# alibaba/graph-learn

Hardware: AMD Instinct MI355X
Metric: sampled-edges/sec + aggregated-vertices/sec (2-hop sample + aggregate per step) (higher is better)
Workload: dtype f32

## Files before the change

### graph-learn_amd/csrc/glx_aggregate.hip

```cpp
#include <float.h>
#include <stdlib.h>
#include <string.h>

#include <atomic>
#include <mutex>
#include <new>
#include <type_traits>

#include "glx_common.h"

namespace {

constexpr int32_t kSegRunMax = 64;


__global__ void glx_seg_reset_kernel(unsigned long long* words) {
  words[0] = 0;
  words[1] = 0;
}

__global__ __launch_bounds__(256) void glx_seg_scan_kernel(const int32_t* __restrict__ seg, int32_t n, int32_t num_segments,
                                                           int32_t f, unsigned long long* __restrict__ words, uint32_t epoch,
                                                           int32_t* __restrict__ seg_start) {
  const int64_t i0 = ((int64_t)blockIdx.x * blockDim.x + threadIdx.x) * 4;
  if (i0 >= n) return;
  int32_t v[4];
  const int32_t m = (n - i0) < 4 ? (int32_t)(n - i0) : 4;
  if (m == 4 && (reinterpret_cast<uintptr_t>(seg) & 15) == 0) {
    const int4 q = *reinterpret_cast<const int4*>(seg + i0);
    v[0] = q.x; v[1] = q.y; v[2] = q.z; v[3] = q.w;
  } else {
    for (int j = 0; j < 4; ++j) v[j] = j < m ? seg[i0 + j] : 0;
  }
  int32_t prev = i0 > 0 ? seg[i0 - 1] : -1;
  if (i0 > 0 && (prev < 0 || prev >= num_segments)) return;
  int32_t quo = f > 0 ? (int32_t)(i0 / f) : 0, rem = f > 0 ? (int32_t)(i0 % f) : 0;
  bool nonuniform = false, incomplete = false;
  int32_t bad_at = n;
  for (int j = 0; j < m; ++j) {
    const int32_t i = (int32_t)i0 + j, cur = v[j];
    if (cur < 0 || cur >= num_segments || cur < prev) {
      bad_at = i;
      break;
    }
    if (cur != prev) {
      if (cur - prev > kSegRunMax) incomplete = true;
      else for (int32_t s = prev + 1; s <= cur; ++s) seg_start[s] = i;
    }
    if (f > 0) {
      nonuniform |= cur != quo;
      if (++rem == f) { rem = 0; ++quo; }
    }
    prev = cur;
  }
  if (bad_at == n && i0 + m == n) {
    if (num_segments - prev > kSegRunMax) incomplete = true;
    else for (int32_t s = prev + 1; s <= num_segments; ++s) seg_start[s] = n;
  }
  const unsigned long long tag = (unsigned long long)epoch << 32;
  if (bad_at < n) atomicMax(&words[0], tag | (uint32_t)(n - bad_at));
  const int32_t level = (incomplete || bad_at < n) ? 2 : (nonuniform ? 1 : 0);
  const uint64_t here = __ballot(true), at2 = __ballot(level == 2), at1 = __ballot(level >= 1);
  const int32_t wave_level = at2 ? 2 : (at1 ? 1 : 0);
  if (wave_level && (threadIdx.x & 63) == (unsigned)(__ffsll((long long)here) - 1)) {
    const unsigned long long mine = tag | (uint32_t)wave_level;
    if (__hip_atomic_load(&words[1], __ATOMIC_RELAXED, __HIP_MEMORY_SCOPE_AGENT) < mine) atomicMax(&words[1], mine);
  }
}

__global__ void glx_seg_fixup_kernel(const int32_t* __restrict__ seg, SegState st, int32_t n, int32_t num_segments,
                                     int32_t* __restrict__ seg_start) {
  if (seg_level(st) != 2) return;
  int32_t s = blockIdx.x * blockDim.x + threadIdx.x;
  if (s > num_segments) return;
  int32_t lo = 0, hi = seg_valid_len(st, n);
  while (lo < hi) {
    int32_t mid = lo + ((hi - lo) >> 1);
    if (seg[mid] < s) lo = mid + 1; else hi = mid;
  }
  seg_start[s] = lo;
}

__global__ void glx_rows_kernel(GlxIdMap map, const int64_t* __restrict__ ids, int64_t n,
                                int32_t* __restrict__ rows) {
  int64_t i = blockIdx.x * (int64_t)blockDim.x + threadIdx.x;
  if (i >= n) return;
  rows[i] = (int32_t)glx_row_of(map, ids[i]);
}


__host__ __device__ __forceinline__ uint16_t glx_f32_to_bf16_bits(uint32_t u) {
  if ((u & 0x7fffffffu) > 0x7f800000u) return 0xFFFF;
  return (uint16_t)((u + 0x7FFFu + ((u >> 16) & 1u)) >> 16);
}
__host__ __device__ __forceinline__ uint16_t glx_f32_to_f16_bits(uint32_t u) {
  const uint32_t sign = (u >> 16) & 0x8000u;
  const uint32_t a = u & 0x7fffffffu;
  if (a > 0x7f800000u) return (uint16_t)(sign | 0x7E00u | ((a >> 13) & 0x3FFu));
  if (a >= 0x477FF000u) return (uint16_t)(sign | 0x7C00u);
  if (a >= 0x38800000u) {
    const uint32_t m = a - 0x38000000u;
    return (uint16_t)(sign | ((m + 0xFFFu + ((m >> 13) & 1u)) >> 13));
  }
  const uint32_t e = a >> 23;
  const uint32_t sh = 126u - e;
  if (sh >= 25u) return (uint16_t)sign;
  const uint32_t mant = (a & 0x7fffffu) | 0x800000u;
  const uint32_t q = mant >> sh, rem = mant & ((1u << sh) - 1u), half = 1u << (sh - 1u);
  return (uint16_t)(sign | (q + ((rem > half || (rem == half && (q & 1u))) ? 1u : 0u)));
}

struct AggArgs {
  const void* X;
  const int64_t* node_ids;
  const int32_t* rows;
  const int32_t* seg_start;
  SegState seg_state;
  float* emb_out;
  int32_t* cnt_out;
  int64_t num_rows;
  int64_t stride;
  int64_t swizzle_rows;
  int32_t dim;
  int32_t num_segments;
  int32_t fanout;
  float default_attr;
  int32_t col0, ncols;
  int32_t store_mode;
  int32_t load_repeats;
  int32_t segs_per_group;
  int32_t xcd_slices;
  int32_t stripe_chunk;
  uint32_t stripe_full;
  const float* X1;
  const float* X2;
  int64_t stride1, swizzle1, stride2;
  int32_t base1, base2;
  int32_t dtype;
};

__device__ __forceinline__ int32_t agg_row_at(const AggArgs& a, int32_t pos) {
  if (a.rows) return a.rows[pos];
  const int64_t id = a.node_ids[pos];
  return (id >= 0 && id < a.num_rows) ? (int32_t)id : -1;
}

template <int NSRC, int DT = GLX_DTYPE_F32>
__device__ __forceinline__ const typename AggElem<DT>::raw* agg_row_ptr(const AggArgs& a, int32_t row) {
  const typename AggElem<DT>::raw* X = static_cast<const typename AggElem<DT>::raw*>(a.X);
  if constexpr (NSRC == 1) {
    return X + glx_swizzle_row(row, a.swizzle_rows) * a.stride;
  } else {
    static_assert(DT == GLX_DTYPE_F32, "the distributed store's row sources are float32");
    if (row < a.base1) return X + glx_swizzle_row(row, a.swizzle_rows) * a.stride;
    if (row < a.base2) return a.X1 + glx_swizzle_row(row - a.base1, a.swizzle1) * a.stride1;
    return a.X2 + (int64_t)(row - a.base2) * a.stride2;
  }
}

template <int OP, int G, int VEC, int U, int NSRC, int DT>
__global__ __launch_bounds__(256) void glx_aggregate_kernel(AggArgs a) {
  typedef float vec_t __attribute__((ext_vector_type(VEC)));
  const int64_t gid = (blockIdx.x * (int64_t)blockDim.x + threadIdx.x) / G;
  const int c = threadIdx.x & (G - 1);
  if (gid >= a.num_segments) return;
  int32_t s0, s1;
  if (a.seg_start && seg_level(a.seg_state) != 0) {
    s0 = a.seg_start[gid];
    s1 = a.seg_start[gid + 1];
  } else {
    s0 = (int32_t)gid * a.fanout;
    s1 = s0 + a.fanout;
  }
  const int32_t n = s1 - s0;
  if (c == 0 && a.col0 == 0) a.cnt_out[gid] = n;
  float* out = a.emb_out + gid * (int64_t)a.dim;
  const int32_t col_end = a.col0 + a.ncols;
  for (int32_t col = a.col0 + c * VEC; col < col_end; col += G * VEC) {
    vec_t acc;
#pragma unroll
    for (int v = 0; v < VEC; ++v) acc[v] = agg_init<OP>();
    for (int32_t base = s0; base < s1; base += U) {
      int32_t row[U];
#pragma unroll
      for (int u = 0; u < U; ++u) row[u] = (base + u < s1) ? agg_row_at(a, base + u) : -2;
      vec_t val[U];
#pragma unroll
      for (int u = 0; u < U; ++u) {
        if (row[u] >= 0) {
          val[u] = agg_load<DT, VEC>(agg_row_ptr<NSRC, DT>(a, row[u]) + col);
        } else {
#pragma unroll
          for (int v = 0; v < VEC; ++v) val[u][v] = a.default_attr;
        }
      }
#pragma unroll
      for (int u = 0; u < U; ++u) {
        if (row[u] != -2) {
#pragma unroll
          for (int v = 0; v < VEC; ++v) acc[v] = agg_combine<OP>(acc[v], val[u][v]);
        }
      }
    }
    if (n == 0) {
#pragma unroll
      for (int v = 0; v < VEC; ++v) acc[v] = a.default_attr;
    } else if (OP == GLX_AGG_MEAN) {
      const float fn = (float)n;
#pragma unroll
      for (int v = 0; v < VEC; ++v) acc[v] = acc[v] / fn;
    }
    *reinterpret_cast<vec_t*>(out + col) = acc;
  }
}

template <int G, int IDR>
__device__ __forceinline__ void agg_chunk_load(const AggArgs& a, int32_t chunk_base, int32_t pos_end, int c,
                                               int32_t (&myrow)[IDR]) {
#pragma unroll
  for (int k = 0; k < IDR; ++k) {
    const int32_t pos = chunk_base + k * G + c;
    myrow[k] = pos < pos_end ? agg_row_at(a, pos) : -1;
  }
}

template <int G, int IDR>
__device__ __forceinline__ int32_t agg_chunk_get(const int32_t (&myrow)[IDR], int32_t idx) {
  if (G == 64) {
    int32_t r = __builtin_amdgcn_readlane(myrow[0], idx & 63);
#pragma unroll
    for (int k = 1; k < IDR; ++k) {
      const int32_t t = __builtin_amdgcn_readlane(myrow[k], idx & 63);
      r = (idx >> 6) == k ? t : r;
// ... 187 lines not shown
          folded = true;
        }
      }
      for (int32_t base = s0; !folded && base < s1; base += U) {
        const int32_t stop = (s1 - base) < U ? s1 : base + U;
        if (stop > chunk_base + kChunk) {
          chunk_base = base;
          agg_chunk_load<G, IDR>(a, chunk_base, pos_end, c, myrow);
        }
        if (stop - base == U) agg_grp_batch<OP, G, VEC, U, NSRC, IDR, true, DT>(a, myrow, base - chunk_base, U, col_ld, acc);
        else agg_grp_batch<OP, G, VEC, U, NSRC, IDR, false, DT>(a, myrow, base - chunk_base, stop - base, col_ld, acc);
      }
      const int32_t n = s1 - s0;
      if (n == 0) {
#pragma unroll
        for (int v = 0; v < VEC; ++v) acc[v] = a.default_attr;
      } else if (OP == GLX_AGG_MEAN) {
        const float fn = (float)n;
#pragma unroll
        for (int v = 0; v < VEC; ++v) acc[v] = acc[v] / fn;
      }
      if (col_ok) {
        float* const dst = a.emb_out + sg * (int64_t)a.dim + col;
        if constexpr (VEC == 8) {
          agg_store4(a.store_mode, dst, acc.lo);
          agg_store4(a.store_mode, dst + 4, acc.hi);
        } else {
          if (a.store_mode == 1) *reinterpret_cast<vec_t*>(dst) = acc;
          else __builtin_nontemporal_store(acc, reinterpret_cast<vec_t*>(dst));
        }
      }
      if (c == 0 && col_pass == 0) a.cnt_out[sg] = n;
    }
  }
}

__device__ __forceinline__ bool agg_nonfinite4(float __attribute__((ext_vector_type(4))) v) {
  const uint32_t e = 0x7f800000u;
  return ((__float_as_uint(v[0]) & e) == e) || ((__float_as_uint(v[1]) & e) == e) || ((__float_as_uint(v[2]) & e) == e) ||
         ((__float_as_uint(v[3]) & e) == e);
}

__device__ __noinline__ float agg_mfma_serial(const float* X, const int64_t* node_ids, const int32_t* rows,
                                              int64_t num_rows, int64_t stride, int64_t swizzle_rows,
                                              float default_attr, int64_t sg, int32_t col, int32_t f) {
  float acc = 0.0f;
  for (int32_t r = 0; r < f; ++r) {
    const int64_t pos = sg * f + r;
    int64_t row;
    if (rows) {
      row = rows[pos];
    } else {
      const int64_t id = node_ids[pos];
      row = (id >= 0 && id < num_rows) ? id : -1;
    }
    const float x = row >= 0 ? X[glx_swizzle_row(row, swizzle_rows) * stride + col] : default_attr;
    acc = acc + x;
  }
  return acc;
}

template <int OP, int NB>
__global__ __launch_bounds__(256) void glx_aggregate_mfma_kernel(AggArgs a) {
  typedef float f4 __attribute__((ext_vector_type(4)));
  constexpr int KC = 32;
  extern __shared__ float tile[];
  constexpr int32_t D = 64 * NB;
  constexpr int32_t pitch = D + 16;
  const int32_t f = a.fanout;
  const int64_t seg0 = (int64_t)blockIdx.x * 16;
  const int32_t nseg = (int32_t)((a.num_segments - seg0) < 16 ? (a.num_segments - seg0) : 16);
  const int64_t id0 = seg0 * f;
  const int32_t nrows = nseg * f;
  const int lane = threadIdx.x & 63;
  const int wave = threadIdx.x >> 6;
  const int m = lane & 15;
  const int kq = lane >> 4;
  f4 acc[NB];
#pragma unroll
  for (int b = 0; b < NB; ++b) acc[b] = f4{0.f, 0.f, 0.f, 0.f};
  constexpr int32_t row_f4 = D / 4;
  constexpr int32_t PT = KC * row_f4 / 256;
  bool nonfinite = false;
  for (int32_t base = 0; base < nrows; base += KC) {
    f4 v[PT];
#pragma unroll
    for (int i = 0; i < PT; ++i) {
      const int32_t p = threadIdx.x + i * 256;
      const int32_t r = p / row_f4;
      const int32_t c4 = p - r * row_f4;
      v[i] = f4{0.f, 0.f, 0.f, 0.f};
      if (base + r < nrows) {
        const int32_t row = agg_row_at(a, (int32_t)(id0 + base + r));
        if (row >= 0) v[i] = *reinterpret_cast<const f4*>(agg_row_ptr<1>(a, row) + c4 * 4);
        else v[i] = f4{a.default_attr, a.default_attr, a.default_attr, a.default_attr};
      }
    }
#pragma unroll
    for (int i = 0; i < PT; ++i) {
      const int32_t p = threadIdx.x + i * 256;
      const int32_t r = p / row_f4;
      const int32_t c4 = p - r * row_f4;
      *reinterpret_cast<f4*>(tile + r * pitch + c4 * 4) = v[i];
      nonfinite |= agg_nonfinite4(v[i]);
    }
    __syncthreads();
#pragma unroll 2
    for (int32_t k4 = 0; k4 < KC; k4 += 4) {
      const int32_t krow = base + k4 + kq;
      const float ind = (krow < nrows && krow / f == m) ? 1.0f : 0.0f;
      const float* brow = tile + (k4 + kq) * pitch + wave * (D / 4) + m;
#pragma unroll
      for (int b = 0; b < NB; ++b) {
        acc[b] = __builtin_amdgcn_mfma_f32_16x16x4f32(ind, brow[b * 16], acc[b], 0, 0, 0);
      }
    }
    __syncthreads();
  }
  const bool refold = __syncthreads_or(nonfinite) != 0;
#pragma unroll
  for (int reg = 0; reg < 4; ++reg) {
    const int32_t srow = kq * 4 + reg;
    if (srow < nseg) {
      float* out = a.emb_out + (seg0 + srow) * (int64_t)D + wave * (D / 4) + m;
#pragma unroll
      for (int b = 0; b < NB; ++b) {
        float v = acc[b][reg];
        if (refold) {
          v = agg_mfma_serial(static_cast<const float*>(a.X), a.node_ids, a.rows, a.num_rows, a.stride, a.swizzle_rows,
                              a.default_attr, seg0 + srow, wave * (D / 4) + m + b * 16, f);
        }
        if (f == 0) v = a.default_attr;
        else if (OP == GLX_AGG_MEAN) v = v / (float)f;
        out[b * 16] = v;
      }
    }
  }
  if (threadIdx.x < nseg) a.cnt_out[seg0 + threadIdx.x] = f;
}

struct AggKnobs {
  std::atomic<int> mfma{0};
  std::atomic<int> unroll{0};
  std::atomic<int> slices{0};
  std::atomic<int> legacy{0};
  std::atomic<int> segs{0};
  std::atomic<int> xcd{0};
  std::atomic<int> occ{0};
  std::atomic<int> store{0};
  std::atomic<int> stripes{-1};
  std::atomic<int> chunk{0};
  std::atomic<int> half_ld16{0};
  std::atomic<int> repeats{0};
};

AggKnobs& agg_knobs() {
  static AggKnobs k;
  static std::once_flag once;
  std::call_once(once, [] {
    auto env = [](const char* name) {
      const char* e = getenv(name);
      return e ? atoi(e) : 0;
    };
    k.mfma = env("GLX_AGG_MFMA");
    k.unroll = env("GLX_AGG_UNROLL");
    k.slices = env("GLX_AGG_SLICES");
    k.legacy = env("GLX_AGG_LEGACY");
    k.segs = env("GLX_AGG_SEGS");
    k.xcd = env("GLX_AGG_XCD_SLICES");
    k.occ = env("GLX_AGG_OCCUPANCY");
    k.store = env("GLX_AGG_STORE");
    if (getenv("GLX_AGG_XCD_STRIPES")) k.stripes = env("GLX_AGG_XCD_STRIPES");
    k.chunk = env("GLX_AGG_XCD_CHUNK");
    k.half_ld16 = env("GLX_AGG_HALF_LD16");
    k.repeats = env("GLX_AGG_REPEATS");
  });
  return k;
}

bool agg_use_mfma(const AggArgs& a, int op) {
  if (agg_knobs().mfma.load(std::memory_order_relaxed) == 0) return false;
  return a.dtype == GLX_DTYPE_F32 && (op == GLX_AGG_SUM || op == GLX_AGG_MEAN) && a.seg_start == nullptr && a.fanout > 0 && a.X1 == nullptr &&
         a.X2 == nullptr && (a.dim == 64 || a.dim == 128 || a.dim == 256) && (a.stride % 4) == 0 &&
         (reinterpret_cast<uintptr_t>(a.X) & 15) == 0;
}

template <int OP>
void launch_agg_mfma(const AggArgs& a, hipStream_t s) {
  const unsigned grid = (unsigned)((a.num_segments + 15) / 16);
  const size_t lds = (size_t)32 * (a.dim + 16) * sizeof(float);
  if (a.dim == 64) glx_aggregate_mfma_kernel<OP, 1><<<grid, 256, lds, s>>>(a);
  else if (a.dim == 128) glx_aggregate_mfma_kernel<OP, 2><<<grid, 256, lds, s>>>(a);
  else glx_aggregate_mfma_kernel<OP, 4><<<grid, 256, lds, s>>>(a);
}

template <int OP, int G, int VEC, int NSRC, int DT>
void launch_agg_g(const AggArgs& a, hipStream_t s) {
  const int64_t threads = (int64_t)a.num_segments * G;
  const unsigned grid = (unsigned)((threads + 255) / 256);
  constexpr bool kWide = VEC == 4 && G >= 32;
  glx_aggregate_kernel<OP, G, VEC, kWide ? 6 : 8, NSRC, DT><<<grid, 256, 0, s>>>(a);
}

int agg_grp_unroll(int32_t fanout, int32_t avg_len) {
  static const int kU[] = {6, 8, 10, 12, 15};
  const int want = agg_knobs().unroll.load(std::memory_order_relaxed);
  for (int u : kU) {
    if (u == want) return u;
  }
  const int32_t f = fanout > 0 ? fanout : (avg_len > 0 ? avg_len : 10);
  int best = 10, best_batches = INT32_MAX;
  for (int u : kU) {
    const int batches = (f + u - 1) / u;
    if (batches < best_batches) {
      best = u;
      best_batches = batches;
    }
  }
  return best;
}

constexpr int32_t kAggSkipMinLen = 16;

template <int OP, int G, int VEC, int NSRC, int IDR, int DT>
void launch_agg_grp(AggArgs a, int32_t num_ids, hipStream_t s) {
  const int32_t avg = a.num_segments > 0 ? (int32_t)(num_ids / a.num_segments) : 0;
  int32_t S = 1;
  const int want = agg_knobs().segs.load(std::memory_order_relaxed);
  constexpr int64_t kElemBytes = sizeof(typename AggElem<DT>::raw);
  if (NSRC == 1 && (int64_t)a.num_rows * a.stride * kElemBytes <= ((int64_t)1 << 30) && a.num_segments >= 3 * 32768) S = 3;
  if (want > 0) S = want;
  if (S > G - 1) S = G - 1;
  if (S < 1) S = 1;
  a.segs_per_group = S;
  a.store_mode = agg_knobs().store.load(std::memory_order_relaxed);
  const int repeats = agg_knobs().repeats.load(std::memory_order_relaxed);
  a.load_repeats = repeats == 1 ? 1 : (repeats == 2 ? 0 : (avg >= kAggSkipMinLen ? 0 : 1));
  const int64_t groups = ((int64_t)a.num_segments + S - 1) / S;
  const int64_t seg_blocks = (groups + (256 / G) - 1) / (256 / G);
  const int32_t nsl = a.xcd_slices > 1 ? a.xcd_slices : 1;
  const int64_t blocks = seg_blocks * nsl;
  const unsigned grid = (unsigned)blocks;
  if (a.stripe_chunk > 0 && nsl < 8) {
    const int64_t span = (int64_t)(8 / nsl) * a.stripe_chunk;
    a.stripe_full = (uint32_t)(seg_blocks / span * span);
  } else {
    a.stripe_chunk = 0;
    a.stripe_full = 0;
  }
  const int occ = agg_knobs().occ.load(std::memory_order_relaxed);
  const size_t lds = (occ >= 3 && occ <= 7) ? (size_t)(160 * 1024 / occ) & ~(size_t)255 : 0;
  switch (agg_grp_unroll(a.seg_start ? 0 : a.fanout, avg)) {
    case 6: glx_aggregate_grp_kernel<OP, G, VEC, 6, NSRC, IDR, DT><<<grid, 256, lds, s>>>(a); break;
    case 8: glx_aggregate_grp_kernel<OP, G, VEC, 8, NSRC, IDR, DT><<<grid, 256, lds, s>>>(a); break;
    case 12: glx_aggregate_grp_kernel<OP, G, VEC, 12, NSRC, IDR, DT><<<grid, 256, lds, s>>>(a); break;
    case 15: glx_aggregate_grp_kernel<OP, G, VEC, 15, NSRC, IDR, DT><<<grid, 256, lds, s>>>(a); break;
    default: glx_aggregate_grp_kernel<OP, G, VEC, 10, NSRC, IDR, DT><<<grid, 256, lds, s>>>(a); break;
  }
}

template <int OP, int VEC, int NSRC, int DT>
void launch_agg_grp_g(const AggArgs& a, int lanes, int32_t num_ids, hipStream_t s) {
  if (lanes >= 64) launch_agg_grp<OP, 64, VEC, NSRC, 1, DT>(a, num_ids, s);
  else if (lanes >= 32) launch_agg_grp<OP, 32, VEC, NSRC, 1, DT>(a, num_ids, s);
  else if (lanes >= 16) launch_agg_grp<OP, 16, VEC, NSRC, 1, DT>(a, num_ids, s);
  else launch_agg_grp<OP, 8, VEC, NSRC, 2, DT>(a, num_ids, s);
}

template <int OP, int NSRC, int DT>
void launch_agg_cols(const AggArgs& a0, int32_t num_ids, int want_xcd, hipStream_t s) {
  AggArgs a = a0;
  bool vec4 = a.dim % 4 == 0 && a.ncols % 4 == 0 && a.col0 % 4 == 0 && (reinterpret_cast<uintptr_t>(a.emb_out) & 15) == 0 &&
              (reinterpret_cast<uintptr_t>(a.X) & 15) == 0 && (a.stride % 4) == 0;
  if (NSRC > 1) {
    vec4 = vec4 && (reinterpret_cast<uintptr_t>(a.X1) & 15) == 0 && (reinterpret_cast<uintptr_t>(a.X2) & 15) == 0 &&
           (a.stride1 % 4) == 0 && (a.stride2 % 4) == 0;
  }
  const int ev = (DT != GLX_DTYPE_F32 && agg_knobs().half_ld16.load(std::memory_order_relaxed) != 0) ? 8 : 4;
  const bool wide = vec4 && a.dim % ev == 0 && a.ncols % ev == 0 && a.col0 % ev == 0 && (a.stride % ev) == 0;
  const bool has_rows = NSRC > 1 ? (a.X2 != nullptr || a.base2 > 0) : a.num_rows > 0;
  if (wide && has_rows && a.ncols >= 8 * ev && agg_knobs().legacy.load(std::memory_order_relaxed) == 0) {
    if (want_xcd > 1 && a.col0 == 0 && a.ncols == a.dim && a.dim % (ev * want_xcd) == 0 && a.dim / want_xcd >= 8 * ev) {
      a.xcd_slices = want_xcd;
      a.ncols = a.dim / want_xcd;
    }
    if constexpr (DT != GLX_DTYPE_F32) {
      if (ev == 8) {
        launch_agg_grp_g<OP, 8, NSRC, DT>(a, a.ncols / 8, num_ids, s);
        return;
      }
    }
    launch_agg_grp_g<OP, 4, NSRC, DT>(a, a.ncols / 4, num_ids, s);
    return;
  }
  if (vec4) {
    const int lanes = a.ncols / 4;
    if (lanes >= 64) launch_agg_g<OP, 64, 4, NSRC, DT>(a, s);
    else if (lanes >= 32) launch_agg_g<OP, 32, 4, NSRC, DT>(a, s);
    else if (lanes >= 16) launch_agg_g<OP, 16, 4, NSRC, DT>(a, s);
    else if (lanes >= 8) launch_agg_g<OP, 8, 4, NSRC, DT>(a, s);
    else if (lanes >= 4) launch_agg_g<OP, 4, 4, NSRC, DT>(a, s);
    else if (lanes >= 2) launch_agg_g<OP, 2, 4, NSRC, DT>(a, s);
    else launch_agg_g<OP, 1, 4, NSRC, DT>(a, s);
  } else {
    const int lanes = a.ncols;
    if (lanes >= 64) launch_agg_g<OP, 64, 1, NSRC, DT>(a, s);
    else if (lanes >= 16) launch_agg_g<OP, 16, 1, NSRC, DT>(a, s);
    else if (lanes >= 4) launch_agg_g<OP, 4, 1, NSRC, DT>(a, s);
    else launch_agg_g<OP, 1, 1, NSRC, DT>(a, s);
  }
}

constexpr int32_t kXcdSliceMinIds = 4 << 20;
constexpr int32_t kXcdStripeChunk = 64;

template <int OP, int NSRC, int DT>
void launch_agg_n(const AggArgs& a0, int32_t num_ids, hipStream_t s) {
  AggArgs a = a0;
  a.col0 = 0;
  a.ncols = a.dim;
  a.xcd_slices = 0;
  int stripes = agg_knobs().stripes.load(std::memory_order_relaxed);
  if (stripes < 0) stripes = num_ids >= kXcdSliceMinIds ? 1 : 0;
  int xcd = agg_knobs().xcd.load(std::memory_order_relaxed);
  if (xcd == 0) {
    xcd = (num_ids >= kXcdSliceMinIds && a.dim % 8 == 0 && a.dim >= 128) ? 2 : 1;
    if (xcd == 2 && stripes > 0 && a.dim >= 256) xcd = 1;
  }
  int slices = agg_knobs().slices.load(std::memory_order_relaxed);
  if ((slices != 2 && slices != 4 && slices != 8) || a.dim % (4 * slices) != 0) slices = 1;
  if (xcd != 2 && xcd != 4 && xcd != 8) xcd = 1;
  int chunk = agg_knobs().chunk.load(std::memory_order_relaxed);
  if (chunk <= 0) chunk = kXcdStripeChunk;
  a.stripe_chunk = stripes > 0 ? chunk : 0;
  for (int c = 0; c < slices; ++c) {
    a.ncols = a.dim / slices;
    a.col0 = c * a.ncols;
    launch_agg_cols<OP, NSRC, DT>(a, num_ids, slices == 1 ? xcd : 1, s);
  }
}

template <int OP>
void launch_agg(const AggArgs& a, int32_t num_ids, hipStream_t s) {
  if (a.X1 || a.X2) launch_agg_n<OP, 3, GLX_DTYPE_F32>(a, num_ids, s);
  else if (a.dtype == GLX_DTYPE_BF16) launch_agg_n<OP, 1, GLX_DTYPE_BF16>(a, num_ids, s);
  else if (a.dtype == GLX_DTYPE_F16) launch_agg_n<OP, 1, GLX_DTYPE_F16>(a, num_ids, s);
  else launch_agg_n<OP, 1, GLX_DTYPE_F32>(a, num_ids, s);
}

template <int SRC, int DST>
__global__ void glx_place_rows_kernel(const void* __restrict__ src_v, int64_t num_rows, int32_t dim,
                                      int64_t stride, int64_t swizzle_rows, void* __restrict__ dst_v) {
  typedef typename std::conditional<SRC == GLX_DTYPE_F32, uint32_t, uint16_t>::type src_t;
  typedef typename std::conditional<DST == GLX_DTYPE_F32, uint32_t, uint16_t>::type dst_t;
  const src_t* __restrict__ src = static_cast<const src_t*>(src_v);
  dst_t* __restrict__ dst = static_cast<dst_t*>(dst_v);
  const int64_t total = num_rows * (int64_t)dim;
  const int64_t step = (int64_t)gridDim.x * blockDim.x;
  for (int64_t t = blockIdx.x * (int64_t)blockDim.x + threadIdx.x; t < total; t += step) {
    const int64_t r = t / dim;
    const int32_t c = (int32_t)(t - r * dim);
    dst_t v;
    if constexpr (SRC == DST) v = src[t];
    else if constexpr (DST == GLX_DTYPE_BF16) v = glx_f32_to_bf16_bits(src[t]);
    else v = glx_f32_to_f16_bits(src[t]);
    dst[glx_swizzle_row(r, swizzle_rows) * stride + c] = v;
  }
}

template <int DT>
__global__ __launch_bounds__(256) void glx_lookup_kernel(GlxIdMap map, const void* __restrict__ Xv,
                                                         int64_t stride, int64_t swizzle_rows, int32_t dim, const int64_t* __restrict__ ids,
                                                         int64_t n, float default_attr,
                                                         float* __restrict__ out, int G) {
  const typename AggElem<DT>::raw* __restrict__ X = static_cast<const typename AggElem<DT>::raw*>(Xv);
  const int64_t gid = (blockIdx.x * (int64_t)blockDim.x + threadIdx.x) / G;
  const int c = threadIdx.x % G;
  if (gid >= n) return;
  int64_t row = glx_row_of(map, ids[gid]);
  if (row >= 0) row = glx_swizzle_row(row, swizzle_rows);
  float* o = out + gid * (int64_t)dim;
  bool vec4 = (dim & 3) == 0;
  if constexpr (DT != GLX_DTYPE_F32) vec4 = vec4 && (stride & 3) == 0 && (reinterpret_cast<uintptr_t>(Xv) & 7) == 0;
  if (vec4) {
    for (int32_t col = c * 4; col < dim; col += G * 4) {
      float4 v = make_float4(default_attr, default_attr, default_attr, default_attr);
      if (row >= 0) {
        const float __attribute__((ext_vector_type(4))) q = agg_load<DT, 4>(X + row * stride + col);
        v = make_float4(q[0], q[1], q[2], q[3]);
      }
      *reinterpret_cast<float4*>(o + col) = v;
    }
  } else {
    for (int32_t col = c; col < dim; col += G) o[col] = row >= 0 ? AggElem<DT>::up(X[row * stride + col]) : default_attr;
  }
}

int run_aggregate(AggArgs& a, int op, const int32_t* d_seg, int32_t num_ids, hipStream_t s) {
  GlxKernelTimer timer(GLX_KERNEL_AGGREGATE, s);
  if (agg_use_mfma(a, op)) {
    if (op == GLX_AGG_SUM) launch_agg_mfma<GLX_AGG_SUM>(a, s);
    else launch_agg_mfma<GLX_AGG_MEAN>(a, s);
    timer.stop();
    return GLX_OK;
  }
  switch (op) {
    case GLX_AGG_SUM: launch_agg<GLX_AGG_SUM>(a, num_ids, s); break;
    case GLX_AGG_MEAN: launch_agg<GLX_AGG_MEAN>(a, num_ids, s); break;
    case GLX_AGG_MAX: launch_agg<GLX_AGG_MAX>(a, num_ids, s); break;
    case GLX_AGG_MIN: launch_agg<GLX_AGG_MIN>(a, num_ids, s); break;
    case GLX_AGG_PROD: launch_agg<GLX_AGG_PROD>(a, num_ids, s); break;
    default: break;
  }
  timer.stop();
  return GLX_OK;
}

namespace {
struct SegBuf {
  int dev;
  hipStream_t stream;
  unsigned long long* words;
  uint32_t epoch;
};
constexpr size_t kSegBufsMax = 64;
struct SegWords {
  std::vector<SegBuf> bufs;
  ~SegWords() {
    for (auto& e : bufs) {
      if (hipSetDevice(e.dev) == hipSuccess) (void)hipFree(e.words);
    }
    (void)hipGetLastError();
  }
};
thread_local SegWords g_seg_words;

int seg_words_for(hipStream_t s, unsigned long long** out, uint32_t* epoch) {
  int dev = 0;
  GLX_HIP(hipGetDevice(&dev));
  SegBuf* buf = nullptr;
  for (auto& e : g_seg_words.bufs) {
    if (e.dev == dev && e.stream == s) {
      buf = &e;
      break;
    }
  }
  if (buf == nullptr) {
    if (g_seg_words.bufs.size() >= kSegBufsMax) {
      const SegBuf old = g_seg_words.bufs.front();
      g_seg_words.bufs.erase(g_seg_words.bufs.begin());
      GlxDeviceGuard guard(old.dev);
      (void)hipFree(old.words);
    }
    unsigned long long* p = nullptr;
    GLX_HIP(hipMalloc(&p, 256));
    GLX_HIP(hipMemsetAsync(p, 0, 256, s));
    g_seg_words.bufs.push_back(SegBuf{dev, s, p, 0u});
    buf = &g_seg_words.bufs.back();
  }
  if (++buf->epoch == 0) {
    GLX_HIP(hipMemsetAsync(buf->words, 0, 16, s));
    buf->epoch = 1;
  }
  *out = buf->words;
  *epoch = buf->epoch;
  return GLX_OK;
}
}


int prepare_segments(AggArgs& a, const int32_t* d_seg, int32_t num_ids, int32_t num_segments, int32_t* scratch,
                     hipStream_t s) {
  a.fanout = num_segments > 0 ? num_ids / num_segments : 0;
  memset(&a.seg_state, 0, sizeof(a.seg_state));
  if (d_seg == nullptr) {
    a.seg_start = nullptr;
    return GLX_OK;
  }
  int32_t* seg_start = scratch;
  unsigned long long* words = nullptr;
  SegState st;
  hipStreamCaptureStatus capturing = hipStreamCaptureStatusNone;
  if (hipStreamIsCapturing(s, &capturing) == hipSuccess && capturing != hipStreamCaptureStatusNone) {
    const uintptr_t at = (reinterpret_cast<uintptr_t>(scratch + (size_t)num_segments + 1) + 7) & ~(uintptr_t)7;
    words = reinterpret_cast<unsigned long long*>(at);
    st.epoch = 1;
    glx_seg_reset_kernel<<<1, 1, 0, s>>>(words);
  } else {
    int rc = seg_words_for(s, &words, &st.epoch);
    if (rc != GLX_OK) return rc;
  }
  const int32_t f = (num_segments > 0 && num_ids > 0 && num_ids % num_segments == 0) ? num_ids / num_segments : 0;
  st.words = words;
  st.floor_level = num_ids == 0 ? 2 : (f > 0 ? 0 : 1);
  if (num_ids > 0) {
    glx_seg_scan_kernel<<<(unsigned)(((int64_t)num_ids + 1023) / 1024), 256, 0, s>>>(d_seg, num_ids, num_segments, f, words,
                                                                                   st.epoch, seg_start);
  }
  glx_seg_fixup_kernel<<<(unsigned)((num_segments + 1 + 255) / 256), 256, 0, s>>>(d_seg, st, num_ids, num_segments, seg_start);
  a.seg_start = seg_start;
  a.seg_state = st;
  return GLX_OK;
}

int aggregate_device(const glx_features* f, int op, const int64_t* d_ids, const int32_t* d_seg,
                     int32_t num_ids, int32_t num_segments, float default_attr, float* d_emb,
                     int32_t* d_cnt, hipStream_t s) {
  const bool hashed = f->idmap.any();
  const size_t n_i32 = (size_t)num_segments + 1 + kSegScratchExtra + (hashed ? (size_t)num_ids : 0);
  GlxScratch lease;
  int rc = lease.alloc(n_i32 * sizeof(int32_t), s, 1);
  if (rc != GLX_OK) return rc;
  int32_t* scratch = lease.as<int32_t>();
  int32_t* rows = hashed ? scratch + num_segments + 1 + kSegScratchExtra : nullptr;
  AggArgs a;
  memset(&a, 0, sizeof(a));
  rc = prepare_segments(a, d_seg, num_ids, num_segments, scratch, s);
  if (rc != GLX_OK) return rc;
  if (hashed && num_ids > 0) {
    glx_rows_kernel<<<(unsigned)((num_ids + 255) / 256), 256, 0, s>>>(f->map(), d_ids, num_ids, rows);
  }
  a.X = f->X;
  a.dtype = f->dtype;
  a.node_ids = hashed ? nullptr : d_ids;
  a.rows = rows;
  a.emb_out = d_emb;
  a.cnt_out = d_cnt;
  a.num_rows = f->num_rows;
  a.stride = f->stride;
  a.swizzle_rows = f->swizzle_rows;
  a.dim = f->dim;
  a.num_segments = num_segments;
  a.default_attr = default_attr;
  run_aggregate(a, op, d_seg, num_ids, s);
  GLX_HIP(hipGetLastError());
  return GLX_OK;
}

template <int OP, int VEC>
__global__ __launch_bounds__(256) void glx_agg_stitch_kernel(const float* __restrict__ parts,
                                                             const int32_t* __restrict__ cnts, int32_t P,
                                                             int64_t num_segments, int32_t dim,
                                                             float default_attr, float* __restrict__ out,
                                                             int32_t* __restrict__ cnt_out) {
  const int32_t cols = dim / VEC;
  const int64_t t = blockIdx.x * (int64_t)blockDim.x + threadIdx.x;
  if (t >= num_segments * cols) return;
  const int64_t sg = t / cols;
  const int32_t c0 = (int32_t)(t - sg * cols) * VEC;
  float acc[VEC];
#pragma unroll
  for (int v = 0; v < VEC; ++v) acc[v] = agg_init<OP>();
  int32_t total = 0;
  for (int32_t p = 0; p < P; ++p) {
    const int32_t c = cnts[(int64_t)p * num_segments + sg];
    if (c == 0) continue;
    const float* src = parts + ((int64_t)p * num_segments + sg) * dim + c0;
    float r[VEC];
    if (VEC == 4) {
      const float4 q = *reinterpret_cast<const float4*>(src);
      r[0] = q.x; r[1 % VEC] = q.y; r[2 % VEC] = q.z; r[3 % VEC] = q.w;
    } else {
      r[0] = src[0];
    }
#pragma unroll
    for (int v = 0; v < VEC; ++v) {
      const float x = OP == GLX_AGG_MEAN ? r[v] * (float)c : r[v];
      acc[v] = agg_combine<OP>(acc[v], x);
    }
    total += c;
  }
#pragma unroll
  for (int v = 0; v < VEC; ++v) {
    if (total == 0) acc[v] = default_attr;
    else if (OP == GLX_AGG_MEAN) acc[v] = acc[v] / (float)total;
  }
  float* dst = out + sg * dim + c0;
  if (VEC == 4) *reinterpret_cast<float4*>(dst) = make_float4(acc[0], acc[1 % VEC], acc[2 % VEC], acc[3 % VEC]);
  else dst[0] = acc[0];
  if (c0 == 0) cnt_out[sg] = total;
}

template <int OP>
void launch_agg_stitch(bool vec4, const float* parts, const int32_t* cnts, int32_t P, int64_t sg, int32_t dim,
                       float default_attr, float* out, int32_t* cnt_out, hipStream_t s) {
  const int64_t threads = sg * (vec4 ? dim / 4 : dim);
  const unsigned grid = (unsigned)((threads + 255) / 256);
  if (vec4) glx_agg_stitch_kernel<OP, 4><<<grid, 256, 0, s>>>(parts, cnts, P, sg, dim, default_attr, out, cnt_out);
  else glx_agg_stitch_kernel<OP, 1><<<grid, 256, 0, s>>>(parts, cnts, P, sg, dim, default_attr, out, cnt_out);
}

}

int glx_aggregate_vrows_device(const GlxRowSource* src, int nsrc, int32_t dim, int op, const int32_t* vrows,
                               const int32_t* d_seg, int32_t num_ids, int32_t num_segments, float default_attr,
                               float* d_emb, int32_t* d_cnt, hipStream_t s) {
  GlxScratch lease;
  int rc = lease.alloc(((size_t)num_segments + 1 + kSegScratchExtra) * sizeof(int32_t), s, 1);
  if (rc != GLX_OK) return rc;
  int32_t* scratch = lease.as<int32_t>();
  AggArgs a;
  memset(&a, 0, sizeof(a));
  rc = prepare_segments(a, d_seg, num_ids, num_segments, scratch, s);
  if (rc != GLX_OK) return rc;
  const GlxRowSource none{nullptr, dim, 0, 0};
  const GlxRowSource& s0 = nsrc > 0 ? src[0] : none;
  const GlxRowSource& s1 = nsrc > 1 ? src[1] : none;
  const GlxRowSource& s2 = nsrc > 2 ? src[2] : none;
  a.X = s0.X;
  a.stride = s0.stride;
  a.swizzle_rows = s0.swizzle_rows;
  a.num_rows = s0.rows;
  a.X1 = s1.X;
  a.stride1 = s1.stride;
  a.swizzle1 = s1.swizzle_rows;
  a.X2 = s2.X;
  a.stride2 = s2.stride;
  a.base1 = (int32_t)s0.rows;
  a.base2 = (int32_t)(s0.rows + s1.rows);
  a.node_ids = nullptr;
  a.rows = vrows;
  a.emb_out = d_emb;
  a.cnt_out = d_cnt;
  a.dim = dim;
  a.num_segments = num_segments;
  a.default_attr = default_attr;
  run_aggregate(a, op, d_seg, num_ids, s);
  GLX_HIP(hipGetLastError());
  return GLX_OK;
}

int glx_segments_prepare(const int32_t* d_seg, int32_t num_ids, int32_t num_segments, int32_t* scratch, hipStream_t s,
                         GlxSegments* out) {
  AggArgs a;
  memset(&a, 0, sizeof(a));
  const int rc = prepare_segments(a, d_seg, num_ids, num_segments, scratch, s);
  if (rc != GLX_OK) return rc;
  out->seg_start = a.seg_start;
  out->state = a.seg_state;
  out->fanout = a.fanout;
  return GLX_OK;
}

extern "C" int glx_tune(const char* name, int32_t value) {
  GLX_REQUIRE(name != nullptr, "name is NULL");
  AggKnobs& k = agg_knobs();
  std::atomic<int>* slot = nullptr;
  if (strcmp(name, "agg_mfma") == 0) slot = &k.mfma;
  else if (strcmp(name, "agg_unroll") == 0) slot = &k.unroll;
  else if (strcmp(name, "agg_slices") == 0) slot = &k.slices;
  else if (strcmp(name, "agg_legacy") == 0) slot = &k.legacy;
  else if (strcmp(name, "agg_segs") == 0) slot = &k.segs;
  else if (strcmp(name, "agg_xcd_slices") == 0) slot = &k.xcd;
  else if (strcmp(name, "agg_occupancy") == 0) slot = &k.occ;
  else if (strcmp(name, "agg_store") == 0) slot = &k.store;
  else if (strcmp(name, "agg_xcd_stripes") == 0) slot = &k.stripes;
  else if (strcmp(name, "agg_xcd_chunk") == 0) slot = &k.chunk;
  else if (strcmp(name, "agg_half_ld16") == 0) slot = &k.half_ld16;
  else if (strcmp(name, "agg_repeats") == 0) slot = &k.repeats;
  else if (strcmp(name, "seg_epochs_before_wrap") == 0) {
    GLX_REQUIRE(value >= 0, "seg_epochs_before_wrap must be >= 0");
    for (auto& e : g_seg_words.bufs) e.epoch = 0xffffffffu - (uint32_t)value;
    return GLX_OK;
  }
  if (slot == nullptr) {
    GlxSideKnobs& sk = glx_side_knobs();
    std::atomic<int64_t>* side = nullptr;
    if (strcmp(name, "cond_sequential") == 0) side = &sk.cond_sequential;
    else if (strcmp(name, "dist_no_bitmap") == 0) side = &sk.dist_no_bitmap;
    else if (strcmp(name, "filter_span_cap") == 0) side = &sk.filter_span_cap;
    else if (strcmp(name, "filter_dedup_min_rows") == 0) side = &sk.filter_dedup_min_rows;
    else if (strcmp(name, "idmap_hash_only") == 0) side = &sk.idmap_hash_only;
    else if (strcmp(name, "knn_chunk_rows") == 0) side = &sk.knn_chunk_rows;
    else if (strcmp(name, "knn_query_block") == 0) side = &sk.knn_query_block;
    else if (strcmp(name, "resolve_ids") == 0) side = &sk.resolve_ids;
    else if (strcmp(name, "resolve_blocks") == 0) side = &sk.resolve_blocks;
    else if (strcmp(name, "resolve_set_share") == 0) side = &sk.resolve_set_share;
    else if (strcmp(name, "resolve_peek") == 0) side = &sk.resolve_peek;
    else if (strcmp(name, "resolve_own_first") == 0) side = &sk.resolve_own_first;
    GLX_REQUIRE(side != nullptr, "unknown knob '%s'", name);
    side->store(value, std::memory_order_relaxed);
    return GLX_OK;
  }
  slot->store(value, std::memory_order_relaxed);
  return GLX_OK;
}

extern "C" int glx_features_create(int device, int64_t num_rows, int32_t dim, const float* X,
                                   const int64_t* ids, int ptr_kind, void* stream,
                                   glx_features** out) {
  return glx_features_create_impl(device, num_rows, dim, X, GLX_DTYPE_F32, GLX_DTYPE_F32, ids, ptr_kind, stream, true, out);
}

extern "C" int glx_features_create_ex(int device, int64_t num_rows, int32_t dim, const void* X, int x_dtype,
                                      int store_dtype, const int64_t* ids, int ptr_kind, void* stream,
                                      glx_features** out) {
  return glx_features_create_impl(device, num_rows, dim, X, x_dtype, store_dtype, ids, ptr_kind, stream, true, out);
}

namespace {
bool glx_dtype_known(int dtype) { return dtype == GLX_DTYPE_F32 || dtype == GLX_DTYPE_BF16 || dtype == GLX_DTYPE_F16; }
}

int glx_features_create_impl(int device, int64_t num_rows, int32_t dim, const void* X, int x_dtype, int store_dtype,
                             const int64_t* ids, int ptr_kind, void* stream, bool allow_arithmetic_ids, glx_features** out) {
  GLX_REQUIRE(out != nullptr, "out is NULL");
  *out = nullptr;
  GLX_REQUIRE(num_rows >= 0 && dim > 0, "bad shape [%lld, %d]", (long long)num_rows, dim);
  GLX_REQUIRE(num_rows < INT32_MAX, "num_rows must be < 2^31");
  GLX_REQUIRE(num_rows == 0 || X != nullptr, "X is NULL");
  GLX_REQUIRE(ptr_kind == GLX_PTR_HOST || ptr_kind == GLX_PTR_DEVICE, "bad ptr_kind");
  GLX_REQUIRE(glx_dtype_known(x_dtype), "unknown x_dtype %d", x_dtype);
  GLX_REQUIRE(glx_dtype_known(store_dtype), "unknown store_dtype %d", store_dtype);
  GLX_REQUIRE(x_dtype == store_dtype || x_dtype == GLX_DTYPE_F32,
              "a %s matrix cannot be stored as %s (only float32 input converts)", glx_dtype_name(x_dtype),
              glx_dtype_name(store_dtype));
  int rc = glx_init_device(device);
  if (rc != GLX_OK) return rc;
  GlxDeviceGuard guard(device);
  GLX_REQUIRE(guard.ok, "cannot select device %d", device);
  hipStream_t s = glx_stream(stream);
  glx_features* f = new (std::nothrow) glx_features();
  GLX_REQUIRE(f != nullptr, "out of host memory");
  memset(static_cast<void*>(f), 0, sizeof(*f));
  f->device = device;
  f->num_rows = num_rows;
  f->dim = dim;
  f->dtype = store_dtype;
  f->elem_size = store_dtype == GLX_DTYPE_F32 ? 4 : 2;
  f->owns_x = true;
  int64_t pad = 0;
  if (const char* env = getenv("GLX_FEATURE_ROW_PAD")) pad = atoll(env);
  if (pad < 0 || (pad % 4) != 0) pad = 0;
  f->stride = dim + pad * 4 / f->elem_size;
  f->swizzle_rows = (num_rows >> GLX_SWIZZLE_BITS) << GLX_SWIZZLE_BITS;
  if (const char* env = getenv("GLX_FEATURE_SWIZZLE")) {
    if (atoi(env) == 0) f->swizzle_rows = 0;
  }
  const size_t bytes = (size_t)(num_rows > 0 ? num_rows : 1) * f->stride * f->elem_size;
  hipError_t e = hipMalloc(&f->X, bytes);
  GlxTemp staged;
  if (e == hipSuccess && num_rows > 0) {
    const void* d_src = X;
    const size_t src_bytes = (size_t)num_rows * dim * (x_dtype == GLX_DTYPE_F32 ? 4 : 2);
    if (ptr_kind == GLX_PTR_HOST) {
      e = hipMalloc(&staged.p, src_bytes);
      if (e == hipSuccess) e = hipMemcpyAsync(staged.p, X, src_bytes, hipMemcpyHostToDevice, s);
      d_src = staged.p;
    }
    if (e == hipSuccess) {
      const int64_t total = num_rows * (int64_t)dim;
      int64_t blocks = (total + 255) / 256;
      if (blocks > 65536) blocks = 65536;
      auto place = glx_place_rows_kernel<GLX_DTYPE_F32, GLX_DTYPE_F32>;
      if (store_dtype == GLX_DTYPE_BF16) {
        place = x_dtype == GLX_DTYPE_F32 ? glx_place_rows_kernel<GLX_DTYPE_F32, GLX_DTYPE_BF16>
                                         : glx_place_rows_kernel<GLX_DTYPE_BF16, GLX_DTYPE_BF16>;
      } else if (store_dtype == GLX_DTYPE_F16) {
        place = x_dtype == GLX_DTYPE_F32 ? glx_place_rows_kernel<GLX_DTYPE_F32, GLX_DTYPE_F16>
                                         : glx_place_rows_kernel<GLX_DTYPE_F16, GLX_DTYPE_F16>;
      }
      place<<<(unsigned)blocks, 256, 0, s>>>(d_src, num_rows, dim, f->stride, f->swizzle_rows, f->X);
    }
  }
  int64_t* tmp_ids = nullptr;
  if (e == hipSuccess && ids) {
    const int64_t* d_ids = ids;
    if (ptr_kind == GLX_PTR_HOST) {
      e = hipMalloc(&tmp_ids, (size_t)(num_rows > 0 ? num_rows : 1) * sizeof(int64_t));
      if (e == hipSuccess) e = hipMemcpyAsync(tmp_ids, ids, (size_t)num_rows * sizeof(int64_t), hipMemcpyHostToDevice, s);
      d_ids = tmp_ids;
    }
    if (e == hipSuccess) {
      rc = allow_arithmetic_ids ? glx_idmap_build_auto(d_ids, num_rows, &f->idmap, s) : glx_idmap_build(d_ids, num_rows, &f->idmap, s);
    }
  }
  if (e == hipSuccess && rc == GLX_OK && f->idmap.keys != nullptr) {
    if (tmp_ids) {
      f->knn_row_ids = tmp_ids;
      tmp_ids = nullptr;
    } else {
      e = hipMalloc(&f->knn_row_ids, (size_t)num_rows * sizeof(int64_t));
      if (e == hipSuccess) e = hipMemcpyAsync(f->knn_row_ids, ids, (size_t)num_rows * sizeof(int64_t), hipMemcpyDeviceToDevice, s);
    }
  }
  if (e == hipSuccess) e = hipStreamSynchronize(s);
  if (tmp_ids) (void)hipFree(tmp_ids);
  if (e != hipSuccess || rc != GLX_OK) {
    if (e != hipSuccess) glx_set_error("feature upload failed: %s", hipGetErrorString(e));
    glx_features_destroy(f);
    return e == hipErrorOutOfMemory ? GLX_RESOURCE_EXHAUSTED : (rc != GLX_OK ? rc : GLX_INTERNAL);
  }
  *out = f;
  return GLX_OK;
}

extern "C" int glx_features_view(int device, int64_t num_rows, int32_t dim, const float* X_device,
                                 glx_features** out) {
  return glx_features_view_ex(device, num_rows, dim, X_device, GLX_DTYPE_F32, out);
}

extern "C" int glx_features_view_ex(int device, int64_t num_rows, int32_t dim, const void* X_device, int dtype,
                                    glx_features** out) {
  GLX_REQUIRE(out != nullptr, "out is NULL");
  *out = nullptr;
  GLX_REQUIRE(num_rows >= 0 && dim > 0, "bad shape [%lld, %d]", (long long)num_rows, dim);
  GLX_REQUIRE(num_rows < INT32_MAX, "num_rows must be < 2^31");
  GLX_REQUIRE(num_rows == 0 || X_device != nullptr, "X is NULL");
  GLX_REQUIRE(glx_dtype_known(dtype), "unknown dtype %d", dtype);
  int rc = glx_init_device(device);
  if (rc != GLX_OK) return rc;
  glx_features* f = new (std::nothrow) glx_features();
// ... 134 lines not shown
```

Measured before the change: 9.129 billion.

## Make segment scan persistent with multi-tile loads and batched fixup searches

Replaces the one-thread-per-4-ids segment scan with a grid-stride persistent kernel capped at a few workgroups per CU. Each thread loads four tiles up front, gets the previous element by wave shuffle instead of a global reload, uses a fast path for runs that step by at most one, and carries the quotient/remainder counters incrementally instead of dividing. Atomics are reduced to one per wave after a shuffle-min of the bad index. The fixup kernel is also capped in grid size and interleaves four binary searches per thread to overlap memory latency. The old kernel is kept behind an env/tune knob. This adds complexity and some risk in the per-lane carry and boundary logic.

```diff
diff --git a/graph-learn_amd/csrc/glx_aggregate.hip b/graph-learn_amd/csrc/glx_aggregate.hip
--- a/graph-learn_amd/csrc/glx_aggregate.hip
+++ b/graph-learn_amd/csrc/glx_aggregate.hip
@@ -19,9 +19,153 @@
   words[1] = 0;
 }
 
-__global__ __launch_bounds__(256) void glx_seg_scan_kernel(const int32_t* __restrict__ seg, int32_t n, int32_t num_segments,
-                                                           int32_t f, unsigned long long* __restrict__ words, uint32_t epoch,
-                                                           int32_t* __restrict__ seg_start) {
+constexpr int kSegScanThreads = 256;
+constexpr int kSegScanLoads = 4;
+constexpr int32_t kSegScanSpan = kSegScanThreads * 4;
+constexpr int32_t kSegScanTile = kSegScanSpan * kSegScanLoads;
+constexpr int kSegScanWgPerCu = 8;
+
+__device__ __forceinline__ void seg_counters_advance(uint32_t& quo, uint32_t& rem, uint32_t dq, uint32_t dr, uint32_t f) {
+  quo += dq;
+  rem += dr;
+  if (rem >= f) {
+    rem -= f;
+    ++quo;
+  }
+}
+
+struct SegScanCarry {
+  uint32_t quo, rem, span_q, span_r, wrap_q, wrap_r;
+  int32_t level, bad_at;
+};
+
+template <bool WHOLE>
+__device__ __forceinline__ void seg_scan_tile(const int32_t* __restrict__ seg, int32_t n, int32_t num_segments, int32_t f,
+                                              int64_t t0, int lane, SegScanCarry& c, int32_t* __restrict__ seg_start) {
+  const uint32_t uf = (uint32_t)f;
+  int32_t v[kSegScanLoads][4], below[kSegScanLoads];
+#pragma unroll
+  for (int L = 0; L < kSegScanLoads; ++L) {
+    const int64_t i0 = t0 + L * kSegScanSpan + threadIdx.x * 4;
+    if (WHOLE) {
+      const int4 q = *reinterpret_cast<const int4*>(seg + i0);
+      v[L][0] = q.x; v[L][1] = q.y; v[L][2] = q.z; v[L][3] = q.w;
+    } else {
+#pragma unroll
+      for (int j = 0; j < 4; ++j) v[L][j] = i0 + j < n ? seg[i0 + j] : 0;
+    }
+    below[L] = (lane == 0 && i0 > 0 && i0 < n) ? seg[i0 - 1] : -1;
+  }
+#pragma unroll
+  for (int L = 0; L < kSegScanLoads; ++L) {
+    const int64_t i0 = t0 + L * kSegScanSpan + threadIdx.x * 4;
+    const int32_t m = i0 >= n ? 0 : ((n - i0) < 4 ? (int32_t)(n - i0) : 4);
+    const int32_t from_lane = __shfl_up(v[L][3], 1);
+    int32_t prev = lane == 0 ? below[L] : from_lane;
+    const bool live = m > 0 && !(i0 > 0 && (prev < 0 || prev >= num_segments));
+    const uint32_t d0 = (uint32_t)v[L][0] - (uint32_t)prev, d1 = (uint32_t)v[L][1] - (uint32_t)v[L][0],
+                   d2 = (uint32_t)v[L][2] - (uint32_t)v[L][1], d3 = (uint32_t)v[L][3] - (uint32_t)v[L][2];
+    const bool plain = (uint32_t)prev < (uint32_t)num_segments && (uint32_t)v[L][3] < (uint32_t)num_segments &&
+                       (d0 | d1 | d2 | d3) <= 1u && i0 + 4 < n;
+    if (plain) {
+      const int32_t i = (int32_t)i0;
+      if (d0) seg_start[v[L][0]] = i;
+      if (d1) seg_start[v[L][1]] = i + 1;
+      if (d2) seg_start[v[L][2]] = i + 2;
+      if (d3) seg_start[v[L][3]] = i + 3;
+      if (f > 0) {
+        uint32_t q = c.quo, r = c.rem;
+        bool nonuniform = false;
+#pragma unroll
+        for (int j = 0; j < 4; ++j) {
+          nonuniform |= (uint32_t)v[L][j] != q;
+          const bool wraps = ++r == uf;
+          q += wraps ? 1u : 0u;
+          r = wraps ? 0u : r;
+        }
+        if (nonuniform && c.level < 1) c.level = 1;
+      }
+    } else if (live) {
+      uint32_t q = c.quo, r = c.rem;
+      bool nonuniform = false, incomplete = false;
+      int32_t bad = n;
+#pragma unroll
+      for (int j = 0; j < 4; ++j) {
+        if (j >= m) break;
+        const int32_t i = (int32_t)i0 + j, cur = v[L][j];
+        if (cur < 0 || cur >= num_segments || cur < prev) {
+          bad = i;
+          break;
+        }
+        if (cur != prev) {
+          if (cur - prev > kSegRunMax) incomplete = true;
+          else for (int32_t s = prev + 1; s <= cur; ++s) seg_start[s] = i;
+        }
+        if (f > 0) {
+          nonuniform |= (uint32_t)cur != q;
+          if (++r == uf) { r = 0; ++q; }
+        }
+        prev = cur;
+      }
+      if (bad == n && i0 + m == n) {
+        if (num_segments - prev > kSegRunMax) incomplete = true;
+        else for (int32_t s = prev + 1; s <= num_segments; ++s) seg_start[s] = n;
+      }
+      if (bad < c.bad_at) c.bad_at = bad;
+      const int32_t here = (incomplete || bad < n) ? 2 : (nonuniform ? 1 : 0);
+      if (here > c.level) c.level = here;
+    }
+    if (f > 0) {
+      if (L + 1 < kSegScanLoads) seg_counters_advance(c.quo, c.rem, c.span_q, c.span_r, uf);
+      else seg_counters_advance(c.quo, c.rem, c.wrap_q, c.wrap_r, uf);
+    }
+  }
+}
+
+__global__ __launch_bounds__(kSegScanThreads) void glx_seg_scan_kernel(const int32_t* __restrict__ seg, int32_t n,
+                                                                       int32_t num_segments, int32_t f,
+                                                                       unsigned long long* __restrict__ words, uint32_t epoch,
+                                                                       int32_t* __restrict__ seg_start) {
+  const int lane = threadIdx.x & 63;
+  const bool aligned = (reinterpret_cast<uintptr_t>(seg) & 15) == 0;
+  const int64_t stride = (int64_t)gridDim.x * kSegScanTile;
+  SegScanCarry c = {0, 0, 0, 0, 0, 0, 0, n};
+  if (f > 0) {
+    const uint32_t uf = (uint32_t)f;
+    const uint32_t first = (uint32_t)blockIdx.x * (uint32_t)kSegScanTile + threadIdx.x * 4u;
+    const uint32_t wrap = (uint32_t)stride - (uint32_t)((kSegScanLoads - 1) * kSegScanSpan);
+    c.quo = first / uf, c.rem = first % uf;
+    c.span_q = (uint32_t)kSegScanSpan / uf, c.span_r = (uint32_t)kSegScanSpan % uf;
+    c.wrap_q = wrap / uf, c.wrap_r = wrap % uf;
+  }
+  for (int64_t t0 = (int64_t)blockIdx.x * kSegScanTile; t0 < n; t0 += stride) {
+    if (aligned && t0 + kSegScanTile <= n) seg_scan_tile<true>(seg, n, num_segments, f, t0, lane, c, seg_start);
+    else seg_scan_tile<false>(seg, n, num_segments, f, t0, lane, c, seg_start);
+  }
+  const unsigned long long tag = (unsigned long long)epoch << 32;
+  int32_t bad_at = c.bad_at;
+  const uint64_t at2 = __ballot(c.level == 2), at1 = __ballot(c.level >= 1);
+  if (at2) {
+#pragma unroll
+    for (int o = 32; o > 0; o >>= 1) {
+      const int32_t other = __shfl_xor(bad_at, o);
+      if (other < bad_at) bad_at = other;
+    }
+  }
+  const int32_t wave_level = at2 ? 2 : (at1 ? 1 : 0);
+  if (wave_level && lane == 0) {
+    if (bad_at < n) {
+      const unsigned long long mine = tag | (uint32_t)(n - bad_at);
+      if (__hip_atomic_load(&words[0], __ATOMIC_RELAXED, __HIP_MEMORY_SCOPE_AGENT) < mine) atomicMax(&words[0], mine);
+    }
+    const unsigned long long mine = tag | (uint32_t)wave_level;
+    if (__hip_atomic_load(&words[1], __ATOMIC_RELAXED, __HIP_MEMORY_SCOPE_AGENT) < mine) atomicMax(&words[1], mine);
+  }
+}
+
+__global__ __launch_bounds__(256) void glx_seg_scan_parent_kernel(const int32_t* __restrict__ seg, int32_t n, int32_t num_segments,
+                                                                  int32_t f, unsigned long long* __restrict__ words, uint32_t epoch,
+                                                                  int32_t* __restrict__ seg_start) {
   const int64_t i0 = ((int64_t)blockIdx.x * blockDim.x + threadIdx.x) * 4;
   if (i0 >= n) return;
   int32_t v[4];
@@ -68,17 +212,42 @@
   }
 }
 
+constexpr int kSegFixupWgPerCu = 2;
+constexpr int kSegFixupSearches = 4;
 __global__ void glx_seg_fixup_kernel(const int32_t* __restrict__ seg, SegState st, int32_t n, int32_t num_segments,
                                      int32_t* __restrict__ seg_start) {
   if (seg_level(st) != 2) return;
-  int32_t s = blockIdx.x * blockDim.x + threadIdx.x;
-  if (s > num_segments) return;
-  int32_t lo = 0, hi = seg_valid_len(st, n);
-  while (lo < hi) {
-    int32_t mid = lo + ((hi - lo) >> 1);
-    if (seg[mid] < s) lo = mid + 1; else hi = mid;
-  }
-  seg_start[s] = lo;
+  const int32_t valid_len = seg_valid_len(st, n);
+  const int64_t step = (int64_t)gridDim.x * blockDim.x;
+  for (int64_t s0 = (int64_t)blockIdx.x * blockDim.x + threadIdx.x; s0 <= num_segments; s0 += step * kSegFixupSearches) {
+    int32_t lo[kSegFixupSearches], hi[kSegFixupSearches];
+#pragma unroll
+    for (int k = 0; k < kSegFixupSearches; ++k) {
+      lo[k] = 0;
+      hi[k] = s0 + k * step <= num_segments ? valid_len : 0;
+    }
+    bool more = valid_len > 0;
+    while (more) {
+      int32_t mid[kSegFixupSearches], at[kSegFixupSearches];
+#pragma unroll
+      for (int k = 0; k < kSegFixupSearches; ++k) {
+        mid[k] = lo[k] + ((hi[k] - lo[k]) >> 1);
+        at[k] = seg[lo[k] < hi[k] ? mid[k] : 0];
+      }
+      more = false;
+#pragma unroll
+      for (int k = 0; k < kSegFixupSearches; ++k) {
+        if (lo[k] < hi[k]) {
+          if (at[k] < s0 + k * step) lo[k] = mid[k] + 1; else hi[k] = mid[k];
+        }
+        more |= lo[k] < hi[k];
+      }
+    }
+#pragma unroll
+    for (int k = 0; k < kSegFixupSearches; ++k) {
+      if (s0 + k * step <= num_segments) seg_start[s0 + k * step] = lo[k];
+    }
+  }
 }
 
 __global__ void glx_rows_kernel(GlxIdMap map, const int64_t* __restrict__ ids, int64_t n,
@@ -572,6 +741,8 @@
   std::atomic<int> chunk{0};
   std::atomic<int> half_ld16{0};
   std::atomic<int> repeats{0};
+  std::atomic<int> seg_parent{0};
+  std::atomic<int> seg_wgs{0};
 };
 
 AggKnobs& agg_knobs() {
@@ -593,6 +764,8 @@
     if (getenv("GLX_AGG_XCD_STRIPES")) k.stripes = env("GLX_AGG_XCD_STRIPES");
     k.chunk = env("GLX_AGG_XCD_CHUNK");
     k.half_ld16 = env("GLX_AGG_HALF_LD16");
+    k.seg_parent = env("GLX_SEG_SCAN_PARENT");
+    k.seg_wgs = env("GLX_SEG_SCAN_WGS");
     k.repeats = env("GLX_AGG_REPEATS");
   });
   return k;
@@ -886,6 +1059,20 @@
   *epoch = buf->epoch;
   return GLX_OK;
 }
+
+int seg_device_cus(int* out) {
+  static std::atomic<int> known[64];
+  int dev = 0;
+  GLX_HIP(hipGetDevice(&dev));
+  int cus = (dev >= 0 && dev < 64) ? known[dev].load(std::memory_order_relaxed) : 0;
+  if (cus <= 0) {
+    GLX_HIP(hipDeviceGetAttribute(&cus, hipDeviceAttributeMultiprocessorCount, dev));
+    GLX_REQUIRE(cus > 0, "device %d reports %d compute units", dev, cus);
+    if (dev >= 0 && dev < 64) known[dev].store(cus, std::memory_order_relaxed);
+  }
+  *out = cus;
+  return GLX_OK;
+}
 }
 
 
@@ -913,11 +1100,27 @@
   const int32_t f = (num_segments > 0 && num_ids > 0 && num_ids % num_segments == 0) ? num_ids / num_segments : 0;
   st.words = words;
   st.floor_level = num_ids == 0 ? 2 : (f > 0 ? 0 : 1);
-  if (num_ids > 0) {
-    glx_seg_scan_kernel<<<(unsigned)(((int64_t)num_ids + 1023) / 1024), 256, 0, s>>>(d_seg, num_ids, num_segments, f, words,
-                                                                                   st.epoch, seg_start);
-  }
-  glx_seg_fixup_kernel<<<(unsigned)((num_segments + 1 + 255) / 256), 256, 0, s>>>(d_seg, st, num_ids, num_segments, seg_start);
+  const bool parent = agg_knobs().seg_parent.load(std::memory_order_relaxed) != 0;
+  int64_t fixup_grid = ((int64_t)num_segments + 1 + 255) / 256;
+  if (parent) {
+    if (num_ids > 0) {
+      glx_seg_scan_parent_kernel<<<(unsigned)(((int64_t)num_ids + 1023) / 1024), 256, 0, s>>>(d_seg, num_ids, num_segments, f,
+                                                                                            words, st.epoch, seg_start);
+    }
+  } else {
+    int cus = 0;
+    int rc = seg_device_cus(&cus);
+    if (rc != GLX_OK) return rc;
+    if (num_ids > 0) {
+      int64_t grid = ((int64_t)num_ids + kSegScanTile - 1) / kSegScanTile;
+      if (grid > (int64_t)cus * kSegScanWgPerCu) grid = (int64_t)cus * kSegScanWgPerCu;
+      const int cap = agg_knobs().seg_wgs.load(std::memory_order_relaxed);
+      if (cap > 0 && grid > cap) grid = cap;
+      glx_seg_scan_kernel<<<(unsigned)grid, kSegScanThreads, 0, s>>>(d_seg, num_ids, num_segments, f, words, st.epoch, seg_start);
+    }
+    if (fixup_grid > (int64_t)cus * kSegFixupWgPerCu) fixup_grid = (int64_t)cus * kSegFixupWgPerCu;
+  }
+  glx_seg_fixup_kernel<<<(unsigned)fixup_grid, 256, 0, s>>>(d_seg, st, num_ids, num_segments, seg_start);
   a.seg_start = seg_start;
   a.seg_state = st;
   return GLX_OK;
@@ -1078,6 +1281,8 @@
   else if (strcmp(name, "agg_xcd_chunk") == 0) slot = &k.chunk;
   else if (strcmp(name, "agg_half_ld16") == 0) slot = &k.half_ld16;
   else if (strcmp(name, "agg_repeats") == 0) slot = &k.repeats;
+  else if (strcmp(name, "seg_scan_parent") == 0) slot = &k.seg_parent;
+  else if (strcmp(name, "seg_scan_wgs") == 0) slot = &k.seg_wgs;
   else if (strcmp(name, "seg_epochs_before_wrap") == 0) {
     GLX_REQUIRE(value >= 0, "seg_epochs_before_wrap must be >= 0");
     for (auto& e : g_seg_words.bufs) e.epoch = 0xffffffffu - (uint32_t)value;
```

New measurement: 9.317 billion, median of 6. +2.1%, better.
